# Borx25/CPU-Raytracing-experiments

Measured on AMD Instinct MI355X. Metric: Mray/s (primary+bounce), higher is better.
Workload: dtype f32; 1 GPU; cfg4: 4096x4096 px, S(100000) spheres + SAH BVH, MIS, Policy.max_bounces=9 (primary+8 bounces), 5 buckets, 64 accumulations/step; fixed image, tile rows split over the GPUs; image=4096x4096, spheres=100000, max_bounces=9, buckets=5, parallelism=single GPU, batches_in_flight=1, accumulations_per_batch=63, accumulations_per_batch_limit=63

## Files before the change

cpu-raytracing-experiments_amd/csrc/kernels.hpp:

```cpp
#pragma once
#include <hip/hip_runtime.h>
#include <stdint.h>
#include "device_math.hpp"
#include "hits_wave_map.hpp"
#include "tile_map.hpp"

namespace mirt {

constexpr uint32_t kBlock = 256;
constexpr uint32_t kShadeBlock = 512;
constexpr uint32_t kTraceBlock = 1024;
constexpr uint32_t kLdsStack = 16;
constexpr uint32_t kLdsStackWide = 12;
constexpr uint32_t kLeafBit = 0x80000000u;
constexpr uint32_t kStack = 64;
constexpr uint32_t kDestAccum = 0x80000000u;

struct SceneDev {
	const float4* recs;
	const float4* spheres;
	const int32_t* prim_mat;
	const float4* light_sphere;
	const float4* light_emit;
	const float4* mat_albedo;
// ... 4 lines not shown
	uint32_t lds_spheres;
	uint32_t half_boxes;
	uint32_t wide;
	uint32_t chunk_max;
	uint32_t leaf_batch;
	uint32_t refill_idle;
	uint32_t stack16;
	float ambient[3];
	int32_t hdri_w, hdri_h;
	float hdri_fw, hdri_fh;
	uint32_t has_ambient;
	uint32_t use_bvh;
};

struct StreamBuf {
	float *px, *py, *pz, *dx, *dy, *dz;
	float *tr, *tg, *tb;
	uint32_t* path;
};
struct ShadowBuf {
	float *px, *py, *pz;
	float *dx, *dy, *dz, *tfar;
	float *sr, *sg, *sb;
	float *er, *eg, *eb;
	uint32_t* dest;
};
struct FrameParams {
	CameraParams cam;
	uint32_t h_tiles;
	uint32_t first_tile;
	uint32_t run_tiles;
	uint32_t stride_tiles;
	uint32_t n_pix;
	uint32_t pix_bits;
	uint32_t pix_mask;
	uint32_t acc_base;
	uint32_t batch_n;
	uint32_t max_bounces;
	uint32_t buckets;
	uint32_t mis;
// ... 531 lines not shown
}
MIRT_DI void lens_camera_ray(const FrameParams& fp, const LensParams& lens, uint32_t i, uint32_t& path, float& px, float& py, float& pz, float& dx, float& dy, float& dz) {
	f3 O, D;
	primary_ray(fp, i, path, D.x, D.y, D.z);
	lens_ray(fp.cam, lens, D, fp.acc_base + (path >> fp.pix_bits) + 1u, path_seed(fp, path & fp.pix_mask), fp.max_bounces, O, D);
	px = O.x; py = O.y; pz = O.z; dx = D.x; dy = D.y; dz = D.z;
}
template <bool LENS = false>
__global__ __launch_bounds__(kBlock) void k_raygen(FrameParams fp, StreamBuf out, uint32_t* stream_count, LensParams lens) {
	const uint32_t total = fp.n_pix * fp.batch_n;
	if (blockIdx.x == 0 && threadIdx.x == 0) stream_count[0] = total;
	for (uint32_t i = blockIdx.x * kBlock + threadIdx.x; i < total; i += gridDim.x * kBlock) {
		uint32_t path; float px, py, pz, dx, dy, dz;
		if (LENS) lens_camera_ray(fp, lens, i, path, px, py, pz, dx, dy, dz);
		else { primary_ray(fp, i, path, dx, dy, dz); px = fp.cam.pos[0]; py = fp.cam.pos[1]; pz = fp.cam.pos[2]; }
		out.px[i] = px; out.py[i] = py; out.pz[i] = pz;
		out.dx[i] = dx; out.dy[i] = dy; out.dz[i] = dz;
		out.path[i] = path;
	}
}

template <int MODE, bool COUNT, class LoadRay, class StoreResult>
MIRT_DI void trace_queue(const SceneDev& sc, const TraceLds tl, const Queue& q, uint32_t n, uint32_t* work_next, FatList fat, uint32_t& c_nodes, uint32_t& c_spheres,
                         LoadRay load_ray, StoreResult store_result, const Collect col = Collect{ nullptr, 0.0f, 0u }) {
	if (n == 0) return;
	const bool all = bvh_all_in_lds(sc);
	if (sc.half_boxes && sc.wide) {
		if (!sc.stack16) trace_persistent<MODE, COUNT, false, true, false, true>(sc, tl, q, n, work_next, fat, c_nodes, c_spheres, load_ray, store_result, col);
		else if (all) trace_persistent<MODE, COUNT, true, true, true, true>(sc, tl, q, n, work_next, fat, c_nodes, c_spheres, load_ray, store_result, col);
		else trace_persistent<MODE, COUNT, false, true, true, true>(sc, tl, q, n, work_next, fat, c_nodes, c_spheres, load_ray, store_result, col);
	} else if (sc.half_boxes) {
		if (!sc.stack16) trace_persistent<MODE, COUNT, false, true, false, false>(sc, tl, q, n, work_next, fat, c_nodes, c_spheres, load_ray, store_result, col);
		else if (all) trace_persistent<MODE, COUNT, true, true, true, false>(sc, tl, q, n, work_next, fat, c_nodes, c_spheres, load_ray, store_result, col);
		else trace_persistent<MODE, COUNT, false, true, true, false>(sc, tl, q, n, work_next, fat, c_nodes, c_spheres, load_ray, store_result, col);
	} else {
		if (all) trace_persistent<MODE, COUNT, true, false, false, false>(sc, tl, q, n, work_next, fat, c_nodes, c_spheres, load_ray, store_result, col);
		else trace_persistent<MODE, COUNT, false, false, false, false>(sc, tl, q, n, work_next, fat, c_nodes, c_spheres, load_ray, store_result, col);
	}
}

MIRT_DI size_t contrib_index(uint32_t batch_n, uint32_t pix_bits, uint32_t path) {
	const uint32_t slot = path >> pix_bits;
	const uint32_t pix = path & ((1u << pix_bits) - 1u);
	return ((static_cast<size_t>(pix >> 8) * batch_n + slot) * kTileSize + (pix & 255u)) * 3u;
}
constexpr uint32_t kDestFull = 0x40000000u;
constexpr uint32_t kDestSlot = 0x3fffffffu;
struct ShadowSink {
	const uint32_t* path;
	const float *px, *py, *pz;
	float* contrib;
	uint32_t batch_n, pix_bits;
	uint32_t* occ;
};
MIRT_DI void shadow_origin(const ShadowBuf& sh, const ShadowSink& sink, uint32_t i, float& px, float& py, float& pz) {
	if (sink.occ) { px = sh.px[i]; py = sh.py[i]; pz = sh.pz[i]; return; }
	const uint32_t dw = sh.dest[i];
	if (dw & kDestAccum) { px = sh.px[i]; py = sh.py[i]; pz = sh.pz[i]; }
	else { const uint32_t d = dw & kDestSlot; px = sink.px[d]; py = sink.py[d]; pz = sink.pz[d]; }
}
MIRT_DI void shadow_finish(const ShadowBuf& sh, const ShadowSink& sink, uint32_t i, bool occluded, uint32_t& c_term) {
	if (sink.occ) { sink.occ[i] = occluded ? 1u : 0u; return; }
	const uint32_t dw = sh.dest[i];
	if (dw & kDestAccum) c_term++;
	const bool full = (dw & kDestFull) != 0u;
	if (occluded & !full) return;
	const uint32_t path = (dw & kDestAccum) ? (dw & kDestSlot) : sink.path[dw & kDestSlot];
	float* w = sink.contrib + contrib_index(sink.batch_n, sink.pix_bits, path);
	f3 R{ w[0], w[1], w[2] };
	if (!occluded) { R.x += sh.sr[i]; R.y += sh.sg[i]; R.z += sh.sb[i]; }
	if (full) { R.x += sh.er[i]; R.y += sh.eg[i]; R.z += sh.eb[i]; }
	w[0] = R.x; w[1] = R.y; w[2] = R.z;
}

constexpr int kPrimaryNone = 0, kPrimaryAll = 1, kPrimaryList = 2;
MIRT_DI uint32_t primary_list_ray(const FrameParams& fp, const uint32_t* __restrict__ ov_pix, uint32_t n_ov, float inv_n_ov, uint32_t j) {
	uint32_t k;
	const uint32_t slot = udiv_f(j, n_ov, inv_n_ov, k);
	return slot * fp.n_pix + ov_pix[k];
}
template <bool COUNT, int PRIMARY, bool LENS = false>
__global__ __launch_bounds__(kTraceBlock, 8) void k_trace(SceneDev sc, FrameParams fp,
                                                       StreamBuf in, HitRec* __restrict__ hit_out,
                                                       Queue closest_queue, uint32_t* closest_work,
                                                       ShadowBuf sh, ShadowSink sink,
                                                       Queue shadow_queue, uint32_t* shadow_work, FatList fat_closest, FatList fat_shadow,
// ... 3 lines not shown
	const float inv_n_ov = 1.0f / static_cast<float>(n_ov ? n_ov : 1u);
	if (PRIMARY) closest_queue.n = nullptr;
	const uint32_t nc = PRIMARY == kPrimaryAll ? fp.n_pix * fp.batch_n : PRIMARY == kPrimaryList ? n_ov * fp.batch_n : queue_total(closest_queue), ns = PRIMARY ? 0u : queue_total(shadow_queue);
	if (nc + ns == 0) return;
	if (blockIdx.x == 0 && threadIdx.x == 0) {
		if (nc && PRIMARY != kPrimaryList) atomicAdd(&ctr->rays, static_cast<unsigned long long>(nc));
		if (ns) atomicAdd(&ctr->shadow_rays, static_cast<unsigned long long>(ns));
	}
	uint32_t c_nodes = 0, c_spheres = 0, s_nodes = 0, s_spheres = 0, c_term = 0;
	if (sc.use_bvh && sc.n_recs != 0) {
		if (static_cast<uint64_t>(blockIdx.x) * 64u >= static_cast<uint64_t>(nc) + ns) return;
		const TraceLds tl = stage_bvh(sc, lds);
		{
			auto load_ray = [&](uint32_t i, float& px, float& py, float& pz, float& dx, float& dy, float& dz, float& tf) {
				if (PRIMARY && LENS) { uint32_t path; lens_camera_ray(fp, lens, i, path, px, py, pz, dx, dy, dz); }
				else if (PRIMARY) { uint32_t path; primary_ray(fp, PRIMARY == kPrimaryList ? primary_list_ray(fp, in.path, n_ov, inv_n_ov, i) : i, path, dx, dy, dz); px = fp.cam.pos[0]; py = fp.cam.pos[1]; pz = fp.cam.pos[2]; }
				else { px = in.px[i]; py = in.py[i]; pz = in.pz[i]; dx = in.dx[i]; dy = in.dy[i]; dz = in.dz[i]; }
				tf = MIRT_FLT_MAX;
			};
			auto store_result = [&](uint32_t i, const Trav& t, bool) { const uint32_t o = PRIMARY == kPrimaryList ? primary_list_ray(fp, in.path, n_ov, inv_n_ov, i) : i; hit_out[o] = HitRec{ t.tfar, t.prim }; };
			trace_queue<kClosest, COUNT>(sc, tl, closest_queue, nc, closest_work, fat_closest, c_nodes, c_spheres, load_ray, store_result);
		}
		if (!PRIMARY) {
			auto load_ray = [&](uint32_t i, float& px, float& py, float& pz, float& dx, float& dy, float& dz, float& tf) {
				shadow_origin(sh, sink, i, px, py, pz); dx = sh.dx[i]; dy = sh.dy[i]; dz = sh.dz[i]; tf = sh.tfar[i];
			};
			auto store_result = [&](uint32_t i, const Trav&, bool occluded) { shadow_finish(sh, sink, i, occluded, c_term); };
			trace_queue<kAnyHit, COUNT>(sc, tl, shadow_queue, ns, shadow_work, fat_shadow, s_nodes, s_spheres, load_ray, store_result);
		}
	} else {
		const QueueView qc = PRIMARY ? queue_identity(nc) : queue_view(closest_queue);
		const QueueView qs = PRIMARY ? queue_identity(0u) : queue_view(shadow_queue);
		for (uint32_t base = blockIdx.x * kTraceBlock; base < nc; base += gridDim.x * kTraceBlock) {
			const bool active = base + threadIdx.x < nc;
			const uint32_t i = active ? queue_slot(qc, base, base + threadIdx.x) : 0u;
			float px = 0, py = 0, pz = 0, dx = 1, dy = 1, dz = 1;
			if (active) {
				if (PRIMARY && LENS) { uint32_t path; lens_camera_ray(fp, lens, i, path, px, py, pz, dx, dy, dz); }
				else if (PRIMARY) { uint32_t path; primary_ray(fp, i, path, dx, dy, dz); px = fp.cam.pos[0]; py = fp.cam.pos[1]; pz = fp.cam.pos[2]; }
				else { px = in.px[i]; py = in.py[i]; pz = in.pz[i]; dx = in.dx[i]; dy = in.dy[i]; dz = in.dz[i]; }
			}
			float tfar = MIRT_FLT_MAX;
			int32_t prim = -1;
			if (sc.use_bvh == 0) traverse_brute<false, COUNT>(sc, lds, active, px, py, pz, dx, dy, dz, tfar, prim, c_spheres);
			if (active) hit_out[i] = HitRec{ tfar, prim };
		}
		for (uint32_t base = blockIdx.x * kTraceBlock; base < ns; base += gridDim.x * kTraceBlock) {
			const bool active = base + threadIdx.x < ns;
			const uint32_t i = active ? queue_slot(qs, base, base + threadIdx.x) : 0u;
			float px = 0, py = 0, pz = 0, dx = 1, dy = 1, dz = 1, tfar = 0;
			if (active) { shadow_origin(sh, sink, i, px, py, pz); dx = sh.dx[i]; dy = sh.dy[i]; dz = sh.dz[i]; tfar = sh.tfar[i]; }
			bool occluded = false;
			int32_t dummy = -1;
			if (sc.use_bvh == 0) occluded = traverse_brute<true, COUNT>(sc, lds, active, px, py, pz, dx, dy, dz, tfar, dummy, s_spheres);
			if (active) shadow_finish(sh, sink, i, occluded, c_term);
		}
	}
	wave_sum(c_term, &ctr->terminated);
	if (COUNT) { wave_sum(c_nodes, &ctr->nodes); wave_sum(c_spheres, &ctr->spheres); wave_sum(s_nodes, &ctr->shadow_nodes); wave_sum(s_spheres, &ctr->shadow_spheres); }
}

template <bool COUNT, int PRIMARY, bool LENS = false>
__global__ __launch_bounds__(1024) void k_trace_fat(SceneDev sc, FrameParams fp, StreamBuf in, HitRec* __restrict__ hit_out, FatList fat_closest,
                                                    ShadowBuf sh, ShadowSink sink, FatList fat_shadow, DevCounters* ctr, const uint32_t* ov_count, LensParams lens) {
	__shared__ float s_t[16];
	__shared__ int32_t s_p[16];
	const uint32_t nc = min(*fat_closest.count, fat_closest.capacity), ns = min(*fat_shadow.count, fat_shadow.capacity);
	const uint32_t lane = threadIdx.x & 63u, wave = threadIdx.x >> 6, n_waves = blockDim.x >> 6;
	const uint32_t n_ov = PRIMARY == kPrimaryList ? *ov_count : 0u;
	const float inv_n_ov = 1.0f / static_cast<float>(n_ov ? n_ov : 1u);
	for (uint32_t k = blockIdx.x; k < nc; k += gridDim.x) {
		const uint32_t i = PRIMARY == kPrimaryList ? primary_list_ray(fp, in.path, n_ov, inv_n_ov, fat_closest.rays[k]) : fat_closest.rays[k];
		float px, py, pz, dx, dy, dz;
		if (PRIMARY && LENS) { uint32_t path; lens_camera_ray(fp, lens, i, path, px, py, pz, dx, dy, dz); }
		else if (PRIMARY) { uint32_t path; primary_ray(fp, i, path, dx, dy, dz); px = fp.cam.pos[0]; py = fp.cam.pos[1]; pz = fp.cam.pos[2]; }
		else { px = in.px[i]; py = in.py[i]; pz = in.pz[i]; dx = in.dx[i]; dy = in.dy[i]; dz = in.dz[i]; }
		float tfar = MIRT_FLT_MAX; int32_t prim = -1;
		for (uint32_t p = threadIdx.x; p < sc.n_spheres; p += blockDim.x) sphere_closest(sc.spheres[p], static_cast<int32_t>(p), px, py, pz, dx, dy, dz, tfar, prim);
		for (int off = 32; off > 0; off >>= 1) {
			const float ot = __shfl_down(tfar, off, 64); const int32_t op = __shfl_down(prim, off, 64);
			const bool take = (op >= 0) & ((prim < 0) | (ot < tfar) | ((ot == tfar) & (op < prim)));
			tfar = take ? ot : tfar; prim = take ? op : prim;
		}
		__syncthreads();
		if (lane == 0) { s_t[wave] = tfar; s_p[wave] = prim; }
		__syncthreads();
		if (threadIdx.x == 0) {
			for (uint32_t w = 1; w < n_waves; w++) {
				const float ot = s_t[w]; const int32_t op = s_p[w];
				const bool take = (op >= 0) && ((prim < 0) || (ot < tfar) || ((ot == tfar) && (op < prim)));
				if (take) { tfar = ot; prim = op; }
			}
			hit_out[i] = HitRec{ tfar, prim };
			if (COUNT) atomicAdd(&ctr->spheres, static_cast<unsigned long long>(sc.n_spheres));
		}
	}
	for (uint32_t k = blockIdx.x; k < ns; k += gridDim.x) {
		const uint32_t i = fat_shadow.rays[k];
		float px, py, pz;
		shadow_origin(sh, sink, i, px, py, pz);
		const float dx = sh.dx[i], dy = sh.dy[i], dz = sh.dz[i], tfar = sh.tfar[i];
		bool occ = false;
		for (uint32_t p = threadIdx.x; p < sc.n_spheres && !occ; p += blockDim.x) occ = sphere_occludes(sc.spheres[p], px, py, pz, dx, dy, dz, tfar);
		const int any = __syncthreads_or(occ ? 1 : 0);
		if (threadIdx.x == 0) {
			uint32_t c_term = 0;
			shadow_finish(sh, sink, i, any != 0, c_term);
			if (c_term) atomicAdd(&ctr->terminated, 1ull);
			if (COUNT) atomicAdd(&ctr->shadow_spheres, static_cast<unsigned long long>(sc.n_spheres));
		}
	}
}

template <bool COUNT, bool LENS>
__global__ __launch_bounds__(kTraceBlock, 8) void k_trace_sparse(SceneDev sc, FrameParams fp, const uint32_t* __restrict__ active_pix, uint32_t n_active, HitRec* __restrict__ hit_out,
                                                              uint32_t* work, FatList fat, DevCounters* ctr, LensParams lens) {
// ... 478 lines not shown
```

cpu-raytracing-experiments_amd/csrc/mirt_capi.hip:

```cpp
#include "../../include/mirt.h"
#include "kernels.hpp"
#include "bvh_layout.hpp"
#include "bvh_build.hpp"
#include "lbvh_build.hpp"
#include "noise_host.hpp"

#include <hip/hip_runtime.h>
#include <algorithm>
#include <cstdarg>
#include <cstdint>
#include <cstdio>
#include <cstdlib>
#include <cstring>
#include <string>
#include <vector>

using namespace mirt;

namespace {

thread_local std::string g_create_error;

struct DeviceBuffer {
	void* ptr = nullptr;
// ... 112 lines not shown
};

namespace {

int fail(mirt_ctx* ctx, int code, const char* fmt, ...) {
	char buf[512];
	va_list ap; va_start(ap, fmt); vsnprintf(buf, sizeof buf, fmt, ap); va_end(ap);
	if (ctx) ctx->error = buf; else g_create_error = buf;
	return code;
}
#define HIP_TRY(ctx, expr) do { hipError_t _e = (expr); if (_e != hipSuccess) return fail(ctx, MIRT_ERR_HIP, "%s: %s", #expr, hipGetErrorString(_e)); } while (0)

constexpr uint32_t kMaxBatch = 256;
constexpr uint64_t kBatchRays = 1024ull << 20;
constexpr uint64_t kSerialRays = 96ull << 20;
constexpr size_t kStreamPlanes = 2 * 10 + 2 + 14;
uint32_t pix_bits_of(const mirt_ctx* c) { uint32_t b = 8; while ((1ull << b) < static_cast<uint64_t>(c->n_tiles) * kTileSize) b++; return b; }
uint32_t max_slots(const mirt_ctx* c) {
	const uint64_t n_pix = std::max<uint64_t>(static_cast<uint64_t>(c->n_tiles) * kTileSize, 1);
	const uint64_t by_slots = ((1ull << 30) - 3ull * kSegs * kShadeBlock) / n_pix;
	return static_cast<uint32_t>(std::max<uint64_t>(std::min<uint64_t>(std::min<uint64_t>(kMaxBatch, 1u << (30u - std::min<uint32_t>(pix_bits_of(c), 24u))), by_slots), 1));
}
uint32_t batch_floor(const mirt_ctx* c) { return std::max<uint32_t>(std::min<uint32_t>(c->policy.buckets, 5u), 1u); }
uint32_t batch_limit(const mirt_ctx* c) {
	if (c->policy.max_batch) return std::min(c->policy.max_batch, max_slots(c));
	const uint64_t n_pix = static_cast<uint64_t>(c->n_tiles) * kTileSize;
	if (n_pix == 0) return 1;
	const uint64_t b = std::max<uint64_t>((kBatchRays + n_pix / 2) / n_pix, batch_floor(c));
	return static_cast<uint32_t>(std::min<uint64_t>(std::min<uint64_t>(b, max_slots(c)), std::max<uint32_t>(c->batch_mem_cap, 1u)));
}

// ... 114 lines not shown
		const char* what = "ray streams";
		if (e == hipSuccess) { e = sl.counts.ensure(BatchCounters::words(nb) * sizeof(uint32_t)); what = "queue counters"; }
		if (e == hipSuccess) { e = sl.fat.ensure(2u * kFatCapacity * sizeof(uint32_t)); what = "fat-ray lists"; }
		if (e == hipSuccess) { e = sl.contrib.ensure(acc_bytes); what = "contribution buffer"; }
		if (e != hipSuccess) {
			(void)hipGetLastError();
			if (e == hipErrorOutOfMemory && !c->policy.max_batch && batch_limit(c) > batch_floor(c)) {
				for (PipeSlot& other : c->slots) { other.arena.release(); other.contrib.release(); }
				c->capacity = 0;
				c->batch_mem_cap = std::max(batch_limit(c) / 2, batch_floor(c));
				return ensure_streams(c);
			}
			return fail(c, MIRT_ERR_HIP, "%s (%zu bytes of ray streams per batch in flight): %s", what, planes * plane_bytes, hipGetErrorString(e));
		}
		char* p = sl.arena.as<char>();
		auto take = [&]() { void* r = p; p += plane_bytes; return r; };
		for (int b = 0; b < 2; b++) {
			StreamBuf& s = sl.stream_buf[b];
			s.px = (float*)take(); s.py = (float*)take(); s.pz = (float*)take();
			s.dx = (float*)take(); s.dy = (float*)take(); s.dz = (float*)take();
			s.tr = (float*)take(); s.tg = (float*)take(); s.tb = (float*)take();
			s.path = (uint32_t*)take();
		}
		sl.hit = (HitRec*)take(); (void)take();
		ShadowBuf& h = sl.shadow_buf;
		h.px = (float*)take(); h.py = (float*)take(); h.pz = (float*)take();
		h.dx = (float*)take(); h.dy = (float*)take(); h.dz = (float*)take(); h.tfar = (float*)take();
		h.sr = (float*)take(); h.sg = (float*)take(); h.sb = (float*)take();
		h.er = (float*)take(); h.eg = (float*)take(); h.eb = (float*)take();
		h.dest = (uint32_t*)take();
	}
	c->capacity = cap;
	c->seg_cap = seg_cap;
	c->arena_bounces = nb;
	return MIRT_OK;
}

size_t aov_floats(const mirt_ctx* c) { return c->aov_on ? static_cast<size_t>(c->n_tiles) * kAovPlanes * kTileSize : 0; }
int alloc_aov(mirt_ctx* c) {
	const size_t floats = aov_floats(c);
	HIP_TRY(c, c->aov.ensure(floats * sizeof(float)));
	if (floats) HIP_TRY(c, hipMemsetAsync(c->aov.ptr, 0, floats * sizeof(float), c->stream));
	return MIRT_OK;
}

// ... 143 lines not shown
	DevCounters* ctr;
};
void launch_trace(const mirt_ctx* c, hipStream_t st, const SceneDev& sc, const FrameParams& fp, uint64_t n_rays, bool count, int primary, const TraceLaunch& t, bool lens = false) {
	hipLaunchKernelGGL(lens ? kTraceLens[!count] : kTrace[!count][primary], dim3(trace_grid(c, n_rays)), dim3(kTraceBlock), trace_lds(c), st, sc, fp, t.in, t.hit, t.closest_queue, t.closest_work,
	                   t.sh, t.sink, t.shadow_queue, t.shadow_work, t.fat_closest, t.fat_shadow, t.ctr, c->lens);
	const uint32_t fat_grid = sc.n_spheres > 4096 ? static_cast<uint32_t>(c->n_cu) * 2u : 64u;
	if (sc.use_bvh) hipLaunchKernelGGL(lens ? kTraceFatLens[!count] : kTraceFat[!count][primary], dim3(fat_grid), dim3(1024), 0, st, sc, fp, t.in, t.hit, t.fat_closest, t.sh, t.sink, t.fat_shadow, t.ctr, t.listed_pixels, c->lens);
}

void launch_trace_sparse(const mirt_ctx* c, hipStream_t st, const SceneDev& sc, const FrameParams& fp, uint32_t active_pix, bool count, const TraceLaunch& t, bool lens) {
	const uint32_t* list = c->active_list.as<uint32_t>();
	hipLaunchKernelGGL(kTraceSparse[!count][lens], dim3(trace_grid(c, static_cast<uint64_t>(active_pix) * fp.batch_n)), dim3(kTraceBlock), trace_lds(c), st, sc, fp, list + 1, active_pix, t.hit,
	                   t.closest_work, t.fat_closest, t.ctr, c->lens);
	const uint32_t fat_grid = sc.n_spheres > 4096 ? static_cast<uint32_t>(c->n_cu) * 2u : 64u;
	StreamBuf listed = t.in;
	listed.path = const_cast<uint32_t*>(list + 1);
	if (sc.use_bvh) hipLaunchKernelGGL(lens ? kTraceFatListLens[!count] : kTraceFat[!count][kPrimaryList], dim3(fat_grid), dim3(1024), 0, st, sc, fp, listed, t.hit, t.fat_closest, t.sh, t.sink, t.fat_shadow, t.ctr, list, c->lens);
}

int launch_tile_stream(mirt_ctx* c, hipStream_t st, const SceneDev& sc, const FrameParams& fp, uint32_t batch_n, float* contrib, DevCounters* ctr, bool count) {
	if (!c->gloss_decay_dev_valid) {
		HIP_TRY(c, sync_all(c));
		HIP_TRY(c, c->gloss_decay_dev.ensure(std::max<size_t>(c->gloss_decay.size(), 1) * sizeof(float)));
		if (!c->gloss_decay.empty()) HIP_TRY(c, hipMemcpy(c->gloss_decay_dev.ptr, c->gloss_decay.data(), c->gloss_decay.size() * sizeof(float), hipMemcpyHostToDevice));
		c->gloss_decay_dev_valid = true;
	}
	Bracket t(c, MIRT_K_TRACE, st);
	hipLaunchKernelGGL(kTileStream[c->policy.brdf != 0], dim3(c->n_tiles * batch_n), dim3(kTileSize), 0, st, sc, fp, contrib, ctr, c->mat_ggx.as<float4>(),
	                   c->gloss_decay_dev.as<float>(), static_cast<uint32_t>(c->gloss_decay.size()), count ? 1u : 0u);
	return MIRT_OK;
}
// ... 92 lines not shown
			const bool shadow_pending = fp.mis && bounce > 0;
			const bool lists = bounce == 0 && bundle;
			{ Bracket t(c, MIRT_K_TRACE, st);
			  if (lists) {
			    if (batch_n >= kWaveHitsMinBatch) {
			      const uint64_t runs = static_cast<uint64_t>(fp.n_pix) / kWaveHitsRun;
			      const uint32_t wgrid = static_cast<uint32_t>(std::min<uint64_t>((runs + kWaveHitsWaves - 1) / kWaveHitsWaves, static_cast<uint64_t>(c->n_cu) * 20u));
			      if (sparse) hipLaunchKernelGGL(kPrimaryHitsWaveSparse[!count], dim3(wgrid), dim3(kBlock), 0, st, sc, fp, c->cand.as<uint32_t>(), sl.hit, ctr, tile_frozen, active_pix);
			      else hipLaunchKernelGGL(kPrimaryHitsWave[!count], dim3(wgrid), dim3(kBlock), 0, st, sc, fp, c->cand.as<uint32_t>(), sl.hit, ctr);
			    } else {
			      const uint32_t hgrid = static_cast<uint32_t>(std::min<uint64_t>((static_cast<uint64_t>(fp.n_pix) + kBlock - 1) / kBlock, static_cast<uint64_t>(c->n_cu) * 64u));
			      if (sparse) hipLaunchKernelGGL(kPrimaryHitsSparse[!count], dim3(hgrid), dim3(kBlock), 0, st, sc, fp, c->cand.as<uint32_t>(), sl.hit, ctr, tile_frozen, active_pix);
			      else hipLaunchKernelGGL(kPrimaryHits[!count], dim3(hgrid), dim3(kBlock), 0, st, sc, fp, c->cand.as<uint32_t>(), sl.hit, ctr);
			    }
			  }
			  const ShadowSink sink{ in.path, in.px, in.py, in.pz, contrib, batch_n, fp.pix_bits, nullptr };
			  StreamBuf rays = in;
			  uint32_t* listed_count = (lists && sparse) ? c->listed_active.as<uint32_t>() : cw.listed_pixels();
			  if (lists) rays.path = sparse ? c->listed_active.as<uint32_t>() + 1 : c->cand_listed.as<uint32_t>();
			  const TraceLaunch tl{ rays, sl.hit, lists ? Queue{ listed_count, 0u } : bc.stream_queue(bounce), bc.closest_work(bounce),
			                        sl.shadow_buf, sink, shadow_pending ? bc.shadow_queue(bounce - 1) : bc.empty_queue(), bc.shadow_work(shadow_pending ? bounce - 1 : 0),
			                        bc.fat_closest(bounce, fat_lists), bc.fat_shadow(bounce, fat_lists), lists ? listed_count : nullptr, ctr };
			  if (sparse && bounce == 0 && !lists) launch_trace_sparse(c, st, sc, fp, active_pix, count, tl, lens);
			  else launch_trace(c, st, sc, fp, total, count, lists ? kPrimaryList : bounce == 0 ? kPrimaryAll : kPrimaryNone, tl, bounce == 0 && lens); }
			if (bounce == 0 && c->aov_on) { const int r = launch_first_hit_aov(c, sl, st, sc, fp); if (r) return r; }
			{ Bracket t(c, MIRT_K_SHADE, st);
			  const float decay = bounce < c->gloss_decay.size() ? c->gloss_decay[bounce] : 0.0f;
			  if (sparse && bounce == 0)
			    hipLaunchKernelGGL(kShadeFirstSparse[c->policy.brdf != 0][lens], dim3(sgrid), dim3(kShadeBlock), 0, st, sc, fp, in, sl.hit, out, sl.shadow_buf, bounce,
			                       bc.stream_queue(bounce), bc.stream_queue(bounce + 1), bc.shadow_queue(bounce), contrib, ctr, mat_ggx, decay, c->lens, tile_frozen);
			  else
			    hipLaunchKernelGGL(bounce == 0 && lens ? kShadeLens[c->policy.brdf != 0] : kShade[bounce == 0][c->policy.brdf != 0], dim3(sgrid), dim3(kShadeBlock), 0, st, sc, fp, in, sl.hit, out, sl.shadow_buf, bounce,
			                       bc.stream_queue(bounce), bc.stream_queue(bounce + 1), bc.shadow_queue(bounce), contrib, ctr, mat_ggx, decay, c->lens); }
		}
// ... 189 lines not shown
	s.wide = t.is_wide ? 1u : 0u;
	c->bvh_depth = t.depth;
	for (int k = 0; k < 3; k++) s.ambient[k] = a.ambient_color[k];
	s.hdri_w = static_cast<int32_t>(a.hdri_w); s.hdri_h = static_cast<int32_t>(a.hdri_h);
	s.hdri_fw = static_cast<float>(static_cast<int32_t>(a.hdri_w) - 1);
	s.hdri_fh = static_cast<float>(static_cast<int32_t>(a.hdri_h) - 1);
	{ const float x = a.ambient_color[0], y = a.ambient_color[1], z = a.ambient_color[2];
	  const float m1 = (y < z) ? z : y; const float m0 = (x < m1) ? m1 : x; s.has_ambient = (m0 > 0.0f) ? 1u : 0u; }
}

int debug_trace(mirt_ctx* c, const char* who, size_t n, const float* p_xyz, const float* dir_xyz, const float* tfar, void* result) {
	const bool shadow = tfar != nullptr;
	const size_t result_bytes = n * (shadow ? sizeof(uint32_t) : sizeof(HitRec));
	HIP_TRY(c, hipSetDevice(c->device));
	ScopedBuffer rays, res, cnt, ctr, fat;
	HIP_TRY(c, rays.ensure(n * (shadow ? 7 : 6) * 4)); HIP_TRY(c, res.ensure(result_bytes)); HIP_TRY(c, cnt.ensure(BatchCounters::words(1) * 4));
	HIP_TRY(c, ctr.ensure(sizeof(DevCounters))); HIP_TRY(c, fat.ensure(2u * kFatCapacity * sizeof(uint32_t)));
	float* d = rays.as<float>();
	HIP_TRY(c, hipMemcpy(d, p_xyz, n * 12, hipMemcpyHostToDevice));
	HIP_TRY(c, hipMemcpy(d + 3 * n, dir_xyz, n * 12, hipMemcpyHostToDevice));
	if (shadow) HIP_TRY(c, hipMemcpy(d + 6 * n, tfar, n * 4, hipMemcpyHostToDevice));
	const BatchCounters bc{ cnt.as<uint32_t>(), 1u, 0u };
	const uint32_t n32 = static_cast<uint32_t>(n);
	HIP_TRY(c, hipMemset(cnt.ptr, 0, BatchCounters::words(1) * 4));
	HIP_TRY(c, hipMemcpy(shadow ? bc.shadow_queue(0).n : bc.stream_queue(0).n, &n32, 4, hipMemcpyHostToDevice));
	HIP_TRY(c, hipMemset(ctr.ptr, 0, sizeof(DevCounters)));
	TraceLaunch tl{};
	if (shadow) { tl.sh.px = d; tl.sh.py = d + n; tl.sh.pz = d + 2 * n; tl.sh.dx = d + 3 * n; tl.sh.dy = d + 4 * n; tl.sh.dz = d + 5 * n; tl.sh.tfar = d + 6 * n; tl.sink.occ = res.as<uint32_t>(); }
	else { tl.in.px = d; tl.in.py = d + n; tl.in.pz = d + 2 * n; tl.in.dx = d + 3 * n; tl.in.dy = d + 4 * n; tl.in.dz = d + 5 * n; tl.hit = res.as<HitRec>(); }
	tl.closest_queue = bc.stream_queue(0); tl.closest_work = bc.closest_work(0);
	tl.shadow_queue = bc.shadow_queue(0); tl.shadow_work = bc.shadow_work(0);
	tl.fat_closest = bc.fat_closest(0, fat.as<uint32_t>()); tl.fat_shadow = bc.fat_shadow(0, fat.as<uint32_t>());
	tl.ctr = ctr.as<DevCounters>();
	{ Bracket t(c, MIRT_K_TRACE);
	  launch_trace(c, c->stream, trace_scene(c), FrameParams{}, n, false, kPrimaryNone, tl); }
	hipError_t e = hipGetLastError();
	if (e == hipSuccess) e = hipStreamSynchronize(c->stream);
	if (e == hipSuccess) e = hipMemcpy(result, res.ptr, result_bytes, hipMemcpyDeviceToHost);
	if (e != hipSuccess) return fail(c, MIRT_ERR_HIP, "%s: %s", who, hipGetErrorString(e));
	return MIRT_OK;
}

}

// ... 536 lines not shown
int mirt_get_stream(mirt_ctx* c, void** s) { if (!c || !s) return MIRT_ERR_ARG; *s = c->stream; return MIRT_OK; }

int mirt_debug_raygen(mirt_ctx* c, uint32_t accumulations, float* p_xyz, float* dir_xyz) {
	int r = check_ready(c); if (r) return r;
	if (!p_xyz || !dir_xyz || accumulations == 0) return fail(c, MIRT_ERR_ARG, "bad arguments");
	if (c->n_tiles == 0) return fail(c, MIRT_ERR_STATE, "no tiles owned");
	HIP_TRY(c, hipSetDevice(c->device));
	if ((r = ensure_streams(c))) return r;
	const FrameParams fp = frame_params(c, accumulations - 1, 1);
	const size_t n = fp.n_pix;
	HIP_TRY(c, sync_all(c));
	hipLaunchKernelGGL(lens_on(c) ? k_raygen<true> : k_raygen<false>, dim3(grid_for(c, n)), dim3(kBlock), 0, c->stream, fp, c->slots[0].stream_buf[0], batch_counters(c, c->slots[0]).stream_queue(0).n, c->lens);
	HIP_TRY(c, hipGetLastError());
	HIP_TRY(c, hipStreamSynchronize(c->stream));
	const StreamBuf& s = c->slots[0].stream_buf[0];
	float* srcs[6] = { s.px, s.py, s.pz, s.dx, s.dy, s.dz };
	for (int k = 0; k < 3; k++) {
		HIP_TRY(c, hipMemcpy(p_xyz + k * n, srcs[k], n * 4, hipMemcpyDeviceToHost));
		HIP_TRY(c, hipMemcpy(dir_xyz + k * n, srcs[3 + k], n * 4, hipMemcpyDeviceToHost));
	}
	return MIRT_OK;
}

int mirt_debug_trace_closest(mirt_ctx* c, size_t n, const float* p_xyz, const float* dir_xyz, float* tfar_out, int32_t* prim_out) {
	if (!c) return MIRT_ERR_ARG;
	if (!c->have_scene) return fail(c, MIRT_ERR_STATE, "mirt_set_scene has not been called");
	if (!p_xyz || !dir_xyz || !tfar_out || !prim_out || n == 0 || n >= (1ull << 31)) return fail(c, MIRT_ERR_ARG, "bad arguments");
	std::vector<HitRec> hits(n);
	const int r = debug_trace(c, "debug_trace_closest", n, p_xyz, dir_xyz, nullptr, hits.data());
	if (r == MIRT_OK) for (size_t i = 0; i < n; i++) { tfar_out[i] = hits[i].tfar; prim_out[i] = hits[i].prim; }
	return r;
}

int mirt_debug_trace_shadow(mirt_ctx* c, size_t n, const float* p_xyz, const float* dir_xyz, const float* tfar, uint8_t* occluded_out) {
// ... 87 lines not shown
```

cpu-raytracing-experiments_amd/csrc/shade_body.inc:

```
	const QueueView qin = FIRST ? queue_identity(fp.n_pix * fp.batch_n) : queue_view(in_queue);
	const uint32_t n = qin.pre[kSegs];
	const uint32_t n_chunks = (fp.n_pix + kShadeBlock - 1u) / kShadeBlock;
	const bool last_bounce = !(bounce < fp.max_bounces - 1u);
	const float light_selection_pdf = 1.0f / static_cast<float>(fp.n_lights);
	__shared__ uint32_t append_scratch[72];
	__shared__ uint32_t compact_scratch[17];
	__shared__ uint32_t hit_list[kShadeBlock];
	__shared__ float4 s_albedo[MIRT_MAX_MATERIALS + 1], s_emission[MIRT_MAX_MATERIALS + 1];
	uint32_t c_term = 0, c_drop = 0, parity = 0;
	const uint32_t n_units = n_chunks * fp.first_groups;
	if (FIRST ? blockIdx.x >= n_units : blockIdx.x * kShadeBlock >= n) return;
	for (uint32_t m = threadIdx.x; m < sc.n_mat; m += kShadeBlock) { s_albedo[m] = GGX ? mat_ggx[m] : sc.mat_albedo[m]; s_emission[m] = sc.mat_emission[m]; }
	__syncthreads();

	uint32_t next_slot = 0u; int32_t next_prim = -1;
	if (!FIRST) {
		next_slot = (blockIdx.x * kShadeBlock + threadIdx.x < n) ? queue_slot(qin, blockIdx.x * kShadeBlock, blockIdx.x * kShadeBlock + threadIdx.x) : 0u;
		next_prim = hit_in[next_slot].prim;
	}
	uint32_t unit = blockIdx.x, chunk = 0u, slot_it = 0u, slot_end = 0u, pix = 0u, pix_seed = 0u;
	int32_t pix_x = 0, pix_y = 0;
	bool pix_frozen = false;
	for (uint32_t base = blockIdx.x * kShadeBlock; FIRST ? unit < n_units : base < n; parity ^= 1u) {
		const bool new_unit = FIRST && slot_it == slot_end;
// ... 37 lines not shown
			const uint32_t nb = base + gridDim.x * kShadeBlock;
			next_slot = (nb + threadIdx.x < n) ? queue_slot(qin, nb, nb + threadIdx.x) : 0u;
			next_prim = hit_in[next_slot].prim;
			base = nb;
		}
		{
			if (lane_on) {
				const uint32_t i = my_slot;
				const int32_t prim = my_prim;
				if (prim < 0) {
					if (sc.has_ambient) {
						if (FIRST) {
							const f3 sky = sky_eval(sc, my_D.x, my_D.y, my_D.z);
							W0 = { 0.0f + 1.0f * sky.x, 0.0f + 1.0f * sky.y, 0.0f + 1.0f * sky.z };
						} else {
							const float thr_x = in.tr[i];
							const f3 sky = sky_eval(sc, in.dx[i], in.dy[i], in.dz[i]);
							float* w = contrib + contrib_index(fp.batch_n, fp.pix_bits, in.path[i]);
							w[0] += thr_x * sky.x; w[1] += thr_x * sky.y; w[2] += thr_x * sky.z;
						}
					}
					c_term++;
				} else if (last_bounce) {
					c_drop++;
					if (!FIRST) {
						float* w = contrib + contrib_index(fp.batch_n, fp.pix_bits, in.path[i]);
						w[0] = 0.0f; w[1] = 0.0f; w[2] = 0.0f;
					}
				} else is_hit = true;
			}
		}
		const uint32_t n_hits = FIRST ? 0u : block_compact(is_hit, my_slot, compact_scratch, hit_list);

		bool survive = false, has_shadow = false, terminated = false, has_E = false;
		uint32_t path = 0;
		f3 P{0, 0, 0}, ndir{0, 0, 0}, L{0, 0, 0}, srad{0, 0, 0}, E{0, 0, 0};
		f3 thr{1.0f, 1.0f, 1.0f};
		float light_distance = 0.0f;
		if (FIRST ? is_hit : threadIdx.x < n_hits) {
			const uint32_t i = FIRST ? my_slot : hit_list[threadIdx.x];
			f3 D = my_D;
			path = my_path;
			if (!FIRST) { path = in.path[i]; D = { in.dx[i], in.dy[i], in.dz[i] }; }
			float pdf_in = 0.0f;
			if (!FIRST) {
				thr = { in.tr[i], in.tg[i], in.tb[i] };
				pdf_in = GGX ? 0.0f : MIRT_INV_PI * max_sel(0.0f, D.z);
			}
			const HitRec hrec = FIRST ? HitRec{ my_tfar, my_prim } : hit_in[i];
			const int32_t prim = hrec.prim;
			{
#define SHADE_HIT_ORIGIN (FIRST ? (LENS ? my_O : f3{ fp.cam.pos[0], fp.cam.pos[1], fp.cam.pos[2] }) : f3{ in.px[i], in.py[i], in.pz[i] })
#define SHADE_HIT_ACC (fp.acc_base + (path >> fp.pix_bits) + 1u)
#define SHADE_HIT_SEED (FIRST ? pix_seed : path_seed(fp, path & fp.pix_mask))
#include "shade_hit_body.inc"
			}
		}
		uint32_t slot, sslot;
		block_append2(survive, has_shadow, next_queue, shadow_queue, iteration % kSegs, append_scratch, parity, slot, sslot);
		const bool full = has_shadow & has_E;
		if (survive) {
			out.px[slot] = P.x; out.py[slot] = P.y; out.pz[slot] = P.z;
			out.dx[slot] = ndir.x; out.dy[slot] = ndir.y; out.dz[slot] = ndir.z;
			out.tr[slot] = thr.x; out.tg[slot] = thr.y; out.tb[slot] = thr.z;
			out.path[slot] = path;
		}
		if (has_shadow) {
			if (!survive) { sh.px[sslot] = P.x; sh.py[sslot] = P.y; sh.pz[sslot] = P.z; }
			sh.dx[sslot] = L.x; sh.dy[sslot] = L.y; sh.dz[sslot] = L.z;
			sh.tfar[sslot] = light_distance;
			sh.sr[sslot] = srad.x; sh.sg[sslot] = srad.y; sh.sb[sslot] = srad.z;
			if (full) { sh.er[sslot] = E.x; sh.eg[sslot] = E.y; sh.eb[sslot] = E.z; }
			sh.dest[sslot] = (survive ? slot : (kDestAccum | path)) | (full ? kDestFull : 0u);
		}
		if (has_E & !has_shadow) {
			if (FIRST) W0 = { 0.0f + E.x, 0.0f + E.y, 0.0f + E.z };
			else {
				float* w = contrib + contrib_index(fp.batch_n, fp.pix_bits, path);
				w[0] += E.x; w[1] += E.y; w[2] += E.z;
			}
		}
		if (FIRST && lane_on) {
			float* w = contrib + contrib_index(fp.batch_n, fp.pix_bits, my_path);
			w[0] = W0.x; w[1] = W0.y; w[2] = W0.z;
		}
		c_term += (terminated && !has_shadow) ? 1u : 0u;
	}
	wave_sum(c_term, &ctr->terminated);
// ... 2 lines not shown
```

Measured before the change: 9478 Mray/s.

## Pack ray and shadow streams from SoA planes into float4 AoS records

Replaces the per-component SoA planes for path and shadow ray streams with packed float4/float2 records, so each ray is loaded and stored with a few wide vector accesses instead of many scalar ones. Shadow rays now always store their own origin and the full path in the dest word, which removes the indirection through the continuation stream. The trade-offs are extra padding bytes, always writing shadow origins, and host-side repacking in the standalone trace/readback API paths.

```diff
diff --git a/cpu-raytracing-experiments_amd/csrc/kernels.hpp b/cpu-raytracing-experiments_amd/csrc/kernels.hpp
--- a/cpu-raytracing-experiments_amd/csrc/kernels.hpp
+++ b/cpu-raytracing-experiments_amd/csrc/kernels.hpp
@@ -42,16 +42,16 @@
 };
 
 struct StreamBuf {
-	float *px, *py, *pz, *dx, *dy, *dz;
-	float *tr, *tg, *tb;
-	uint32_t* path;
+	float4* a;
+	float4* b;
+	float2* c;
 };
+MIRT_DI const uint32_t* stream_pixel_list(const StreamBuf& in) { return reinterpret_cast<const uint32_t*>(in.a); }
 struct ShadowBuf {
-	float *px, *py, *pz;
-	float *dx, *dy, *dz, *tfar;
-	float *sr, *sg, *sb;
-	float *er, *eg, *eb;
-	uint32_t* dest;
+	float4* a;
+	float4* b;
+	float4* c;
+	float4* d;
 };
 struct FrameParams {
 	CameraParams cam;
@@ -613,9 +613,8 @@
 		uint32_t path; float px, py, pz, dx, dy, dz;
 		if (LENS) lens_camera_ray(fp, lens, i, path, px, py, pz, dx, dy, dz);
 		else { primary_ray(fp, i, path, dx, dy, dz); px = fp.cam.pos[0]; py = fp.cam.pos[1]; pz = fp.cam.pos[2]; }
-		out.px[i] = px; out.py[i] = py; out.pz[i] = pz;
-		out.dx[i] = dx; out.dy[i] = dy; out.dz[i] = dz;
-		out.path[i] = path;
+		out.a[i] = make_float4(px, py, pz, __uint_as_float(path));
+		out.b[i] = make_float4(dx, dy, dz, 1.0f);
 	}
 }
 
@@ -644,31 +643,26 @@
 	return ((static_cast<size_t>(pix >> 8) * batch_n + slot) * kTileSize + (pix & 255u)) * 3u;
 }
 constexpr uint32_t kDestFull = 0x40000000u;
-constexpr uint32_t kDestSlot = 0x3fffffffu;
+constexpr uint32_t kDestPath = 0x3fffffffu;
 struct ShadowSink {
-	const uint32_t* path;
-	const float *px, *py, *pz;
 	float* contrib;
 	uint32_t batch_n, pix_bits;
 	uint32_t* occ;
 };
-MIRT_DI void shadow_origin(const ShadowBuf& sh, const ShadowSink& sink, uint32_t i, float& px, float& py, float& pz) {
-	if (sink.occ) { px = sh.px[i]; py = sh.py[i]; pz = sh.pz[i]; return; }
-	const uint32_t dw = sh.dest[i];
-	if (dw & kDestAccum) { px = sh.px[i]; py = sh.py[i]; pz = sh.pz[i]; }
-	else { const uint32_t d = dw & kDestSlot; px = sink.px[d]; py = sink.py[d]; pz = sink.pz[d]; }
+MIRT_DI void shadow_ray(const ShadowBuf& sh, uint32_t i, float& px, float& py, float& pz, float& dx, float& dy, float& dz, float& tfar) {
+	const float4 a = sh.a[i], b = sh.b[i];
+	px = a.x; py = a.y; pz = a.z; tfar = a.w; dx = b.x; dy = b.y; dz = b.z;
 }
 MIRT_DI void shadow_finish(const ShadowBuf& sh, const ShadowSink& sink, uint32_t i, bool occluded, uint32_t& c_term) {
 	if (sink.occ) { sink.occ[i] = occluded ? 1u : 0u; return; }
-	const uint32_t dw = sh.dest[i];
+	const uint32_t dw = __float_as_uint(sh.b[i].w);
 	if (dw & kDestAccum) c_term++;
 	const bool full = (dw & kDestFull) != 0u;
 	if (occluded & !full) return;
-	const uint32_t path = (dw & kDestAccum) ? (dw & kDestSlot) : sink.path[dw & kDestSlot];
-	float* w = sink.contrib + contrib_index(sink.batch_n, sink.pix_bits, path);
+	float* w = sink.contrib + contrib_index(sink.batch_n, sink.pix_bits, dw & kDestPath);
 	f3 R{ w[0], w[1], w[2] };
-	if (!occluded) { R.x += sh.sr[i]; R.y += sh.sg[i]; R.z += sh.sb[i]; }
-	if (full) { R.x += sh.er[i]; R.y += sh.eg[i]; R.z += sh.eb[i]; }
+	if (!occluded) { const float4 S = sh.c[i]; R.x += S.x; R.y += S.y; R.z += S.z; }
+	if (full) { const float4 E = sh.d[i]; R.x += E.x; R.y += E.y; R.z += E.z; }
 	w[0] = R.x; w[1] = R.y; w[2] = R.z;
 }
 
@@ -702,16 +696,16 @@
 		{
 			auto load_ray = [&](uint32_t i, float& px, float& py, float& pz, float& dx, float& dy, float& dz, float& tf) {
 				if (PRIMARY && LENS) { uint32_t path; lens_camera_ray(fp, lens, i, path, px, py, pz, dx, dy, dz); }
-				else if (PRIMARY) { uint32_t path; primary_ray(fp, PRIMARY == kPrimaryList ? primary_list_ray(fp, in.path, n_ov, inv_n_ov, i) : i, path, dx, dy, dz); px = fp.cam.pos[0]; py = fp.cam.pos[1]; pz = fp.cam.pos[2]; }
-				else { px = in.px[i]; py = in.py[i]; pz = in.pz[i]; dx = in.dx[i]; dy = in.dy[i]; dz = in.dz[i]; }
+				else if (PRIMARY) { uint32_t path; primary_ray(fp, PRIMARY == kPrimaryList ? primary_list_ray(fp, stream_pixel_list(in), n_ov, inv_n_ov, i) : i, path, dx, dy, dz); px = fp.cam.pos[0]; py = fp.cam.pos[1]; pz = fp.cam.pos[2]; }
+				else { const float4 a = in.a[i], b = in.b[i]; px = a.x; py = a.y; pz = a.z; dx = b.x; dy = b.y; dz = b.z; }
 				tf = MIRT_FLT_MAX;
 			};
-			auto store_result = [&](uint32_t i, const Trav& t, bool) { const uint32_t o = PRIMARY == kPrimaryList ? primary_list_ray(fp, in.path, n_ov, inv_n_ov, i) : i; hit_out[o] = HitRec{ t.tfar, t.prim }; };
+			auto store_result = [&](uint32_t i, const Trav& t, bool) { const uint32_t o = PRIMARY == kPrimaryList ? primary_list_ray(fp, stream_pixel_list(in), n_ov, inv_n_ov, i) : i; hit_out[o] = HitRec{ t.tfar, t.prim }; };
 			trace_queue<kClosest, COUNT>(sc, tl, closest_queue, nc, closest_work, fat_closest, c_nodes, c_spheres, load_ray, store_result);
 		}
 		if (!PRIMARY) {
 			auto load_ray = [&](uint32_t i, float& px, float& py, float& pz, float& dx, float& dy, float& dz, float& tf) {
-				shadow_origin(sh, sink, i, px, py, pz); dx = sh.dx[i]; dy = sh.dy[i]; dz = sh.dz[i]; tf = sh.tfar[i];
+				shadow_ray(sh, i, px, py, pz, dx, dy, dz, tf);
 			};
 			auto store_result = [&](uint32_t i, const Trav&, bool occluded) { shadow_finish(sh, sink, i, occluded, c_term); };
 			trace_queue<kAnyHit, COUNT>(sc, tl, shadow_queue, ns, shadow_work, fat_shadow, s_nodes, s_spheres, load_ray, store_result);
@@ -726,7 +720,7 @@
 			if (active) {
 				if (PRIMARY && LENS) { uint32_t path; lens_camera_ray(fp, lens, i, path, px, py, pz, dx, dy, dz); }
 				else if (PRIMARY) { uint32_t path; primary_ray(fp, i, path, dx, dy, dz); px = fp.cam.pos[0]; py = fp.cam.pos[1]; pz = fp.cam.pos[2]; }
-				else { px = in.px[i]; py = in.py[i]; pz = in.pz[i]; dx = in.dx[i]; dy = in.dy[i]; dz = in.dz[i]; }
+				else { const float4 a = in.a[i], b = in.b[i]; px = a.x; py = a.y; pz = a.z; dx = b.x; dy = b.y; dz = b.z; }
 			}
 			float tfar = MIRT_FLT_MAX;
 			int32_t prim = -1;
@@ -737,7 +731,7 @@
 			const bool active = base + threadIdx.x < ns;
 			const uint32_t i = active ? queue_slot(qs, base, base + threadIdx.x) : 0u;
 			float px = 0, py = 0, pz = 0, dx = 1, dy = 1, dz = 1, tfar = 0;
-			if (active) { shadow_origin(sh, sink, i, px, py, pz); dx = sh.dx[i]; dy = sh.dy[i]; dz = sh.dz[i]; tfar = sh.tfar[i]; }
+			if (active) shadow_ray(sh, i, px, py, pz, dx, dy, dz, tfar);
 			bool occluded = false;
 			int32_t dummy = -1;
 			if (sc.use_bvh == 0) occluded = traverse_brute<true, COUNT>(sc, lds, active, px, py, pz, dx, dy, dz, tfar, dummy, s_spheres);
@@ -758,11 +752,11 @@
 	const uint32_t n_ov = PRIMARY == kPrimaryList ? *ov_count : 0u;
 	const float inv_n_ov = 1.0f / static_cast<float>(n_ov ? n_ov : 1u);
 	for (uint32_t k = blockIdx.x; k < nc; k += gridDim.x) {
-		const uint32_t i = PRIMARY == kPrimaryList ? primary_list_ray(fp, in.path, n_ov, inv_n_ov, fat_closest.rays[k]) : fat_closest.rays[k];
+		const uint32_t i = PRIMARY == kPrimaryList ? primary_list_ray(fp, stream_pixel_list(in), n_ov, inv_n_ov, fat_closest.rays[k]) : fat_closest.rays[k];
 		float px, py, pz, dx, dy, dz;
 		if (PRIMARY && LENS) { uint32_t path; lens_camera_ray(fp, lens, i, path, px, py, pz, dx, dy, dz); }
 		else if (PRIMARY) { uint32_t path; primary_ray(fp, i, path, dx, dy, dz); px = fp.cam.pos[0]; py = fp.cam.pos[1]; pz = fp.cam.pos[2]; }
-		else { px = in.px[i]; py = in.py[i]; pz = in.pz[i]; dx = in.dx[i]; dy = in.dy[i]; dz = in.dz[i]; }
+		else { const float4 a = in.a[i], b = in.b[i]; px = a.x; py = a.y; pz = a.z; dx = b.x; dy = b.y; dz = b.z; }
 		float tfar = MIRT_FLT_MAX; int32_t prim = -1;
 		for (uint32_t p = threadIdx.x; p < sc.n_spheres; p += blockDim.x) sphere_closest(sc.spheres[p], static_cast<int32_t>(p), px, py, pz, dx, dy, dz, tfar, prim);
 		for (int off = 32; off > 0; off >>= 1) {
@@ -785,9 +779,8 @@
 	}
 	for (uint32_t k = blockIdx.x; k < ns; k += gridDim.x) {
 		const uint32_t i = fat_shadow.rays[k];
-		float px, py, pz;
-		shadow_origin(sh, sink, i, px, py, pz);
-		const float dx = sh.dx[i], dy = sh.dy[i], dz = sh.dz[i], tfar = sh.tfar[i];
+		float px, py, pz, dx, dy, dz, tfar;
+		shadow_ray(sh, i, px, py, pz, dx, dy, dz, tfar);
 		bool occ = false;
 		for (uint32_t p = threadIdx.x; p < sc.n_spheres && !occ; p += blockDim.x) occ = sphere_occludes(sc.spheres[p], px, py, pz, dx, dy, dz, tfar);
 		const int any = __syncthreads_or(occ ? 1 : 0);
diff --git a/cpu-raytracing-experiments_amd/csrc/mirt_capi.hip b/cpu-raytracing-experiments_amd/csrc/mirt_capi.hip
--- a/cpu-raytracing-experiments_amd/csrc/mirt_capi.hip
+++ b/cpu-raytracing-experiments_amd/csrc/mirt_capi.hip
@@ -150,7 +150,7 @@
 constexpr uint32_t kMaxBatch = 256;
 constexpr uint64_t kBatchRays = 1024ull << 20;
 constexpr uint64_t kSerialRays = 96ull << 20;
-constexpr size_t kStreamPlanes = 2 * 10 + 2 + 14;
+constexpr size_t kStreamPlanes = 2 * 10 + 2 + 16;
 uint32_t pix_bits_of(const mirt_ctx* c) { uint32_t b = 8; while ((1ull << b) < static_cast<uint64_t>(c->n_tiles) * kTileSize) b++; return b; }
 uint32_t max_slots(const mirt_ctx* c) {
 	const uint64_t n_pix = std::max<uint64_t>(static_cast<uint64_t>(c->n_tiles) * kTileSize, 1);
@@ -295,21 +295,14 @@
 			return fail(c, MIRT_ERR_HIP, "%s (%zu bytes of ray streams per batch in flight): %s", what, planes * plane_bytes, hipGetErrorString(e));
 		}
 		char* p = sl.arena.as<char>();
-		auto take = [&]() { void* r = p; p += plane_bytes; return r; };
+		auto take = [&](size_t n_planes) { void* r = p; p += n_planes * plane_bytes; return r; };
 		for (int b = 0; b < 2; b++) {
 			StreamBuf& s = sl.stream_buf[b];
-			s.px = (float*)take(); s.py = (float*)take(); s.pz = (float*)take();
-			s.dx = (float*)take(); s.dy = (float*)take(); s.dz = (float*)take();
-			s.tr = (float*)take(); s.tg = (float*)take(); s.tb = (float*)take();
-			s.path = (uint32_t*)take();
+			s.a = (float4*)take(4); s.b = (float4*)take(4); s.c = (float2*)take(2);
 		}
-		sl.hit = (HitRec*)take(); (void)take();
+		sl.hit = (HitRec*)take(2);
 		ShadowBuf& h = sl.shadow_buf;
-		h.px = (float*)take(); h.py = (float*)take(); h.pz = (float*)take();
-		h.dx = (float*)take(); h.dy = (float*)take(); h.dz = (float*)take(); h.tfar = (float*)take();
-		h.sr = (float*)take(); h.sg = (float*)take(); h.sb = (float*)take();
-		h.er = (float*)take(); h.eg = (float*)take(); h.eb = (float*)take();
-		h.dest = (uint32_t*)take();
+		h.a = (float4*)take(4); h.b = (float4*)take(4); h.c = (float4*)take(4); h.d = (float4*)take(4);
 	}
 	c->capacity = cap;
 	c->seg_cap = seg_cap;
@@ -483,7 +476,7 @@
 	                   t.closest_work, t.fat_closest, t.ctr, c->lens);
 	const uint32_t fat_grid = sc.n_spheres > 4096 ? static_cast<uint32_t>(c->n_cu) * 2u : 64u;
 	StreamBuf listed = t.in;
-	listed.path = const_cast<uint32_t*>(list + 1);
+	listed.a = reinterpret_cast<float4*>(const_cast<uint32_t*>(list + 1));
 	if (sc.use_bvh) hipLaunchKernelGGL(lens ? kTraceFatListLens[!count] : kTraceFat[!count][kPrimaryList], dim3(fat_grid), dim3(1024), 0, st, sc, fp, listed, t.hit, t.fat_closest, t.sh, t.sink, t.fat_shadow, t.ctr, list, c->lens);
 }
 
@@ -606,10 +599,10 @@
 			      else hipLaunchKernelGGL(kPrimaryHits[!count], dim3(hgrid), dim3(kBlock), 0, st, sc, fp, c->cand.as<uint32_t>(), sl.hit, ctr);
 			    }
 			  }
-			  const ShadowSink sink{ in.path, in.px, in.py, in.pz, contrib, batch_n, fp.pix_bits, nullptr };
+			  const ShadowSink sink{ contrib, batch_n, fp.pix_bits, nullptr };
 			  StreamBuf rays = in;
 			  uint32_t* listed_count = (lists && sparse) ? c->listed_active.as<uint32_t>() : cw.listed_pixels();
-			  if (lists) rays.path = sparse ? c->listed_active.as<uint32_t>() + 1 : c->cand_listed.as<uint32_t>();
+			  if (lists) rays.a = reinterpret_cast<float4*>(sparse ? c->listed_active.as<uint32_t>() + 1 : c->cand_listed.as<uint32_t>());
 			  const TraceLaunch tl{ rays, sl.hit, lists ? Queue{ listed_count, 0u } : bc.stream_queue(bounce), bc.closest_work(bounce),
 			                        sl.shadow_buf, sink, shadow_pending ? bc.shadow_queue(bounce - 1) : bc.empty_queue(), bc.shadow_work(shadow_pending ? bounce - 1 : 0),
 			                        bc.fat_closest(bounce, fat_lists), bc.fat_shadow(bounce, fat_lists), lists ? listed_count : nullptr, ctr };
@@ -829,20 +822,23 @@
 	const size_t result_bytes = n * (shadow ? sizeof(uint32_t) : sizeof(HitRec));
 	HIP_TRY(c, hipSetDevice(c->device));
 	ScopedBuffer rays, res, cnt, ctr, fat;
-	HIP_TRY(c, rays.ensure(n * (shadow ? 7 : 6) * 4)); HIP_TRY(c, res.ensure(result_bytes)); HIP_TRY(c, cnt.ensure(BatchCounters::words(1) * 4));
+	HIP_TRY(c, rays.ensure(n * 2 * sizeof(float4))); HIP_TRY(c, res.ensure(result_bytes)); HIP_TRY(c, cnt.ensure(BatchCounters::words(1) * 4));
 	HIP_TRY(c, ctr.ensure(sizeof(DevCounters))); HIP_TRY(c, fat.ensure(2u * kFatCapacity * sizeof(uint32_t)));
-	float* d = rays.as<float>();
-	HIP_TRY(c, hipMemcpy(d, p_xyz, n * 12, hipMemcpyHostToDevice));
-	HIP_TRY(c, hipMemcpy(d + 3 * n, dir_xyz, n * 12, hipMemcpyHostToDevice));
-	if (shadow) HIP_TRY(c, hipMemcpy(d + 6 * n, tfar, n * 4, hipMemcpyHostToDevice));
+	float4* d = rays.as<float4>();
+	{ std::vector<float4> rec(2 * n);
+	  for (size_t i = 0; i < n; i++) {
+	    rec[i] = make_float4(p_xyz[i], p_xyz[n + i], p_xyz[2 * n + i], shadow ? tfar[i] : 0.0f);
+	    rec[n + i] = make_float4(dir_xyz[i], dir_xyz[n + i], dir_xyz[2 * n + i], 0.0f);
+	  }
+	  HIP_TRY(c, hipMemcpy(d, rec.data(), 2 * n * sizeof(float4), hipMemcpyHostToDevice)); }
 	const BatchCounters bc{ cnt.as<uint32_t>(), 1u, 0u };
 	const uint32_t n32 = static_cast<uint32_t>(n);
 	HIP_TRY(c, hipMemset(cnt.ptr, 0, BatchCounters::words(1) * 4));
 	HIP_TRY(c, hipMemcpy(shadow ? bc.shadow_queue(0).n : bc.stream_queue(0).n, &n32, 4, hipMemcpyHostToDevice));
 	HIP_TRY(c, hipMemset(ctr.ptr, 0, sizeof(DevCounters)));
 	TraceLaunch tl{};
-	if (shadow) { tl.sh.px = d; tl.sh.py = d + n; tl.sh.pz = d + 2 * n; tl.sh.dx = d + 3 * n; tl.sh.dy = d + 4 * n; tl.sh.dz = d + 5 * n; tl.sh.tfar = d + 6 * n; tl.sink.occ = res.as<uint32_t>(); }
-	else { tl.in.px = d; tl.in.py = d + n; tl.in.pz = d + 2 * n; tl.in.dx = d + 3 * n; tl.in.dy = d + 4 * n; tl.in.dz = d + 5 * n; tl.hit = res.as<HitRec>(); }
+	if (shadow) { tl.sh.a = d; tl.sh.b = d + n; tl.sink.occ = res.as<uint32_t>(); }
+	else { tl.in.a = d; tl.in.b = d + n; tl.hit = res.as<HitRec>(); }
 	tl.closest_queue = bc.stream_queue(0); tl.closest_work = bc.closest_work(0);
 	tl.shadow_queue = bc.shadow_queue(0); tl.shadow_work = bc.shadow_work(0);
 	tl.fat_closest = bc.fat_closest(0, fat.as<uint32_t>()); tl.fat_shadow = bc.fat_shadow(0, fat.as<uint32_t>());
@@ -1409,10 +1405,12 @@
 	HIP_TRY(c, hipGetLastError());
 	HIP_TRY(c, hipStreamSynchronize(c->stream));
 	const StreamBuf& s = c->slots[0].stream_buf[0];
-	float* srcs[6] = { s.px, s.py, s.pz, s.dx, s.dy, s.dz };
-	for (int k = 0; k < 3; k++) {
-		HIP_TRY(c, hipMemcpy(p_xyz + k * n, srcs[k], n * 4, hipMemcpyDeviceToHost));
-		HIP_TRY(c, hipMemcpy(dir_xyz + k * n, srcs[3 + k], n * 4, hipMemcpyDeviceToHost));
+	std::vector<float4> rec(2 * n);
+	HIP_TRY(c, hipMemcpy(rec.data(), s.a, n * sizeof(float4), hipMemcpyDeviceToHost));
+	HIP_TRY(c, hipMemcpy(rec.data() + n, s.b, n * sizeof(float4), hipMemcpyDeviceToHost));
+	for (size_t i = 0; i < n; i++) {
+		p_xyz[i] = rec[i].x; p_xyz[n + i] = rec[i].y; p_xyz[2 * n + i] = rec[i].z;
+		dir_xyz[i] = rec[n + i].x; dir_xyz[n + i] = rec[n + i].y; dir_xyz[2 * n + i] = rec[n + i].z;
 	}
 	return MIRT_OK;
 }
diff --git a/cpu-raytracing-experiments_amd/csrc/shade_body.inc b/cpu-raytracing-experiments_amd/csrc/shade_body.inc
--- a/cpu-raytracing-experiments_amd/csrc/shade_body.inc
+++ b/cpu-raytracing-experiments_amd/csrc/shade_body.inc
@@ -75,9 +75,10 @@
 							const f3 sky = sky_eval(sc, my_D.x, my_D.y, my_D.z);
 							W0 = { 0.0f + 1.0f * sky.x, 0.0f + 1.0f * sky.y, 0.0f + 1.0f * sky.z };
 						} else {
-							const float thr_x = in.tr[i];
-							const f3 sky = sky_eval(sc, in.dx[i], in.dy[i], in.dz[i]);
-							float* w = contrib + contrib_index(fp.batch_n, fp.pix_bits, in.path[i]);
+							const float4 b = in.b[i];
+							const float thr_x = b.w;
+							const f3 sky = sky_eval(sc, b.x, b.y, b.z);
+							float* w = contrib + contrib_index(fp.batch_n, fp.pix_bits, __float_as_uint(in.a[i].w));
 							w[0] += thr_x * sky.x; w[1] += thr_x * sky.y; w[2] += thr_x * sky.z;
 						}
 					}
@@ -85,7 +86,7 @@
 				} else if (last_bounce) {
 					c_drop++;
 					if (!FIRST) {
-						float* w = contrib + contrib_index(fp.batch_n, fp.pix_bits, in.path[i]);
+						float* w = contrib + contrib_index(fp.batch_n, fp.pix_bits, __float_as_uint(in.a[i].w));
 						w[0] = 0.0f; w[1] = 0.0f; w[2] = 0.0f;
 					}
 				} else is_hit = true;
@@ -102,16 +103,20 @@
 			const uint32_t i = FIRST ? my_slot : hit_list[threadIdx.x];
 			f3 D = my_D;
 			path = my_path;
-			if (!FIRST) { path = in.path[i]; D = { in.dx[i], in.dy[i], in.dz[i] }; }
+			f3 O_in{0, 0, 0};
 			float pdf_in = 0.0f;
 			if (!FIRST) {
-				thr = { in.tr[i], in.tg[i], in.tb[i] };
+				const float4 a = in.a[i], b = in.b[i];
+				const float2 c = in.c[i];
+				O_in = { a.x, a.y, a.z }; path = __float_as_uint(a.w);
+				D = { b.x, b.y, b.z };
+				thr = { b.w, c.x, c.y };
 				pdf_in = GGX ? 0.0f : MIRT_INV_PI * max_sel(0.0f, D.z);
 			}
 			const HitRec hrec = FIRST ? HitRec{ my_tfar, my_prim } : hit_in[i];
 			const int32_t prim = hrec.prim;
 			{
-#define SHADE_HIT_ORIGIN (FIRST ? (LENS ? my_O : f3{ fp.cam.pos[0], fp.cam.pos[1], fp.cam.pos[2] }) : f3{ in.px[i], in.py[i], in.pz[i] })
+#define SHADE_HIT_ORIGIN (FIRST ? (LENS ? my_O : f3{ fp.cam.pos[0], fp.cam.pos[1], fp.cam.pos[2] }) : O_in)
 #define SHADE_HIT_ACC (fp.acc_base + (path >> fp.pix_bits) + 1u)
 #define SHADE_HIT_SEED (FIRST ? pix_seed : path_seed(fp, path & fp.pix_mask))
 #include "shade_hit_body.inc"
@@ -121,18 +126,15 @@
 		block_append2(survive, has_shadow, next_queue, shadow_queue, iteration % kSegs, append_scratch, parity, slot, sslot);
 		const bool full = has_shadow & has_E;
 		if (survive) {
-			out.px[slot] = P.x; out.py[slot] = P.y; out.pz[slot] = P.z;
-			out.dx[slot] = ndir.x; out.dy[slot] = ndir.y; out.dz[slot] = ndir.z;
-			out.tr[slot] = thr.x; out.tg[slot] = thr.y; out.tb[slot] = thr.z;
-			out.path[slot] = path;
+			out.a[slot] = make_float4(P.x, P.y, P.z, __uint_as_float(path));
+			out.b[slot] = make_float4(ndir.x, ndir.y, ndir.z, thr.x);
+			out.c[slot] = make_float2(thr.y, thr.z);
 		}
 		if (has_shadow) {
-			if (!survive) { sh.px[sslot] = P.x; sh.py[sslot] = P.y; sh.pz[sslot] = P.z; }
-			sh.dx[sslot] = L.x; sh.dy[sslot] = L.y; sh.dz[sslot] = L.z;
-			sh.tfar[sslot] = light_distance;
-			sh.sr[sslot] = srad.x; sh.sg[sslot] = srad.y; sh.sb[sslot] = srad.z;
-			if (full) { sh.er[sslot] = E.x; sh.eg[sslot] = E.y; sh.eb[sslot] = E.z; }
-			sh.dest[sslot] = (survive ? slot : (kDestAccum | path)) | (full ? kDestFull : 0u);
+			sh.a[sslot] = make_float4(P.x, P.y, P.z, light_distance);
+			sh.b[sslot] = make_float4(L.x, L.y, L.z, __uint_as_float(path | (survive ? 0u : kDestAccum) | (full ? kDestFull : 0u)));
+			sh.c[sslot] = make_float4(srad.x, srad.y, srad.z, 0.0f);
+			if (full) sh.d[sslot] = make_float4(E.x, E.y, E.z, 0.0f);
 		}
 		if (has_E & !has_shadow) {
 			if (FIRST) W0 = { 0.0f + E.x, 0.0f + E.y, 0.0f + E.z };
```

Measured after the change: 9818 Mray/s, median of 6. +3.6%, better.
